# SynthAIr/T-VQ-VAE-TrajGen

Hardware: AMD Instinct MI355X
Metric: stage1+stage2 train steps/sec on synthetic (B,C,T) trajectories, 1/2/4/8 GPU (higher is better)
Workload: dtype fp32; 1 GPU; stage1 VQ-VAE + stage2 MaskGIT joint train step, per-GPU batch (B=256,C=6,T=256), K=512, configs/config.yaml architecture; global_batch=256, seq_len=256, parallelism=dp1, launch=hipgraph

## Files before the change

t-vq-vae-trajgen_amd/csrc/tvq_conv_wgrad.hip:

```cpp
#include "tvq_conv_core.h"
#include "tvq_conv_internal.h"
#include "tvq_gemm.h"
#include "tvq_reduce.h"

#include <algorithm>
#include <vector>

namespace tvq {

template <int KH, int KW, int SW, bool REPL, int TN, int TK, int WN, int WK>
__global__ __launch_bounds__(256) void conv_wgrad_kernel(const float* __restrict__ G,
                                                        const float* __restrict__ in,
                                                        float* __restrict__ slab, ConvGeom g,
                                                        int pos_per_split, int kcols) {
  constexpr int BK = 16;
  constexpr int KK = KH * KW;
  constexpr int FN = TN / WN / 16;
  constexpr int FK = TK / WK / 16;
  constexpr int SA = ((TN + 31) / 32) * 32 + 16;
  constexpr int SB = ((TK + 31) / 32) * 32 + 16;
  constexpr int A_PER = TN * BK / 256;
  constexpr int B_PER = TK * BK / 256;
  static_assert(A_PER >= 1 && B_PER >= 1, "tile too small");
  __shared__ float As[BK * SA];
  __shared__ float Bs[BK * SB];

  const int tid = threadIdx.x, lane = tid & 63, wid = tid >> 6;
  const int wn = wid % WN, wk = wid / WN;
  const int n0 = blockIdx.y * TN;
  const int kp0 = blockIdx.x * TK;
  const int p_begin = blockIdx.z * pos_per_split;
  const int p_end = min(g.Mpos, p_begin + pos_per_split);

  const int kk_t = tid % BK;
  const int a_nbase = tid / BK;
  const int b_kbase = tid / BK;
  int bc_off[B_PER], bkh[B_PER], bkw[B_PER];
  unsigned bmask = 0u, bones = 0u;
#pragma unroll
  for (int j = 0; j < B_PER; ++j) {
    const int kp = kp0 + b_kbase + j * 16;
    const int c = kp / KK, r = kp - c * KK;
    bkh[j] = r / KW - g.oph;
    bkw[j] = r - (r / KW) * KW - g.opw;
    bc_off[j] = (kp < g.Kred) ? c * g.Hin * g.Win : 0;
    if (kp < g.Kred) bmask |= 1u << j;
    if (kp == g.Kred && kp < kcols) bones |= 1u << j;
  }

  float ra[A_PER], rb[B_PER];
  auto load_tile = [&](int p0) {
    const int p = p0 + kk_t;
    const bool pv = p < p_end;
    int b = 0, h = 0, w = 0;
    if (pv) {
      const uint32_t bh = fdiv((uint32_t)p, g.fd_wo);
      w = p - (int)bh * g.Wo;
      b = (int)fdiv((uint32_t)p, g.fd_hwo);
      h = (int)bh - b * g.Hout;
    }
    const float* gb = G + (((int64_t)b * g.N) * g.Hout + h) * g.Wo + w;
#pragma unroll
    for (int j = 0; j < A_PER; ++j) {
      const int n = n0 + a_nbase + j * 16;
      ra[j] = (pv && n < g.N) ? gb[(int64_t)n * g.Hout * g.Wo] : 0.f;
    }
    const float* inb = in + (int64_t)b * g.C * g.Hin * g.Win;
#pragma unroll
    for (int j = 0; j < B_PER; ++j) {
      float v = (pv && (bones >> j & 1u)) ? 1.0f : 0.f;
      if (pv && (bmask >> j & 1u)) {
        int hi = h + bkh[j], wi = w * SW + bkw[j];
        bool ok = true;
        if (REPL) {
          hi = hi < 0 ? 0 : (hi >= g.Hin ? g.Hin - 1 : hi);
          wi = wi < 0 ? 0 : (wi >= g.Win ? g.Win - 1 : wi);
        } else {
          ok = hi >= 0 && hi < g.Hin && wi >= 0 && wi < g.Win;
        }
        if (ok) v = inb[bc_off[j] + (int64_t)hi * g.Win + wi];
      }
      rb[j] = v;
    }
  };
  auto store_tile = [&]() {
#pragma unroll
    for (int j = 0; j < A_PER; ++j) As[kk_t * SA + ((a_nbase + j * 16) ^ (kk_t & 14))] = ra[j];
#pragma unroll
    for (int j = 0; j < B_PER; ++j) Bs[kk_t * SB + ((b_kbase + j * 16) ^ (kk_t & 14))] = rb[j];
  };

  floatx4 acc[FN][FK];
#pragma unroll
  for (int i = 0; i < FN; ++i)
#pragma unroll
    for (int j = 0; j < FK; ++j) acc[i][j] = floatx4{0.f, 0.f, 0.f, 0.f};
  const int r16 = lane & 15, g4 = lane >> 4;
  if (p_begin < p_end) {
    load_tile(p_begin);
    for (int p0 = p_begin; p0 < p_end; p0 += BK) {
      __syncthreads();
      store_tile();
      __syncthreads();
      if (p0 + BK < p_end) load_tile(p0 + BK);
#pragma unroll
      for (int kk = 0; kk < BK; kk += 4) {
        float af[FN], bf[FK];
        const int swz = r16 ^ ((kk & 12) | (g4 & 2));
#pragma unroll
        for (int i = 0; i < FN; ++i) af[i] = As[(kk + g4) * SA + (wn * FN + i) * 16 + swz];
#pragma unroll
        for (int j = 0; j < FK; ++j) bf[j] = Bs[(kk + g4) * SB + (wk * FK + j) * 16 + swz];
#pragma unroll
        for (int i = 0; i < FN; ++i)
#pragma unroll
          for (int j = 0; j < FK; ++j) acc[i][j] = mfma16x16x4(af[i], bf[j], acc[i][j]);
      }
    }
  }
  float* sl = slab + (int64_t)blockIdx.z * g.N * kcols;
#pragma unroll
  for (int i = 0; i < FN; ++i)
#pragma unroll
    for (int j = 0; j < FK; ++j)
#pragma unroll
      for (int r = 0; r < 4; ++r) {
        const int n = n0 + (wn * FN + i) * 16 + 4 * g4 + r;
        const int kp = kp0 + (wk * FK + j) * 16 + r16;
        if (n < g.N && kp < kcols) sl[(int64_t)n * kcols + kp] = acc[i][j][r];
      }
}
__device__ __forceinline__ void chan_sum_final_one(const float* part, int chunks, int c,
                                                   float* out, int accumulate) {
  float s = 0.f;
  for (int i = 0; i < chunks; ++i) s += ld_wt(part + (int64_t)c * chunks + i);
  out[c] = accumulate ? out[c] + s : s;
}
__global__ __launch_bounds__(256) void chan_sum_partial_kernel(const float* __restrict__ x, int B,
                                                               int C, int HW, int ipc, int chunks,
                                                               int vec, float* __restrict__ part,
                                                               int* __restrict__ cnt,
                                                               float* __restrict__ out,
                                                               int accumulate) {
  __shared__ float red[4];
  const int c = blockIdx.x, ch = blockIdx.y;
  const int b0 = ch * ipc, b1 = min(B, b0 + ipc);
  float s = 0.f;
  if (vec) {
    const int hw4 = HW >> 2, n4 = (b1 - b0) * hw4;
    for (int i0 = threadIdx.x; i0 < n4; i0 += 256 * 4) {
      floatx4 v[4];
#pragma unroll
      for (int u = 0; u < 4; ++u) {
        const int i = i0 + u * 256;
        const int bb = b0 + (i < n4 ? i : 0) / hw4, q = (i < n4 ? i : 0) % hw4;
        v[u] = *reinterpret_cast<const floatx4*>(x + ((int64_t)bb * C + c) * HW + 4 * q);
      }
#pragma unroll
      for (int u = 0; u < 4; ++u)
        if (i0 + u * 256 < n4) s += (v[u][0] + v[u][1]) + (v[u][2] + v[u][3]);
    }
  } else {
    const int n = (b1 - b0) * HW;
    for (int i = threadIdx.x; i < n; i += 256) {
      const int bb = b0 + i / HW, p = i % HW;
      s += x[((int64_t)bb * C + c) * HW + p];
    }
  }
  s = block_sum(s, red);
  if (threadIdx.x == 0) st_wt(part + (int64_t)c * chunks + ch, s);
  if (cnt && last_block(cnt + c, chunks) && threadIdx.x < 64) {
    float t = threadIdx.x < chunks ? ld_wt(part + (int64_t)c * chunks + threadIdx.x) : 0.f;
    t = wave_sum(t);
    if (threadIdx.x == 0) out[c] = accumulate ? out[c] + t : t;
  }
}
__global__ void chan_sum_final_kernel(const float* __restrict__ part, int C, int chunks,
                                      float* __restrict__ out, int accumulate) {
  const int c = blockIdx.x * blockDim.x + threadIdx.x;
  if (c >= C) return;
  chan_sum_final_one(part, chunks, c, out, accumulate);
}

struct WHaloGeom {
  Div16 dv_hw, dv_wp, dv_gst;
  int B, C, Hin, Win, N, Hout, Wo;
  int oh, ow, HP, WP, PS;
  int P, GST, CB;
  int Kred, kcols;
  int ips;
};

template <int KH, int KW, int SW, bool REPL, int FN>
__global__ __launch_bounds__(256) void conv_wgrad_halo_kernel(const float* __restrict__ G,
                                                             const float* __restrict__ in,
                                                             float* __restrict__ slab,
                                                             WHaloGeom g) {
  constexpr int KK = KH * KW;
  constexpr int NB = FN * 16;
  extern __shared__ float smem[];
  float* Gs = smem;
  float* Hs = smem + NB * g.GST;
  const int tid = threadIdx.x, lane = tid & 63, wid = tid >> 6;
  const int s = blockIdx.x;
  const int n0 = blockIdx.y * NB;
  const int c0 = blockIdx.z * g.CB;
  const int cbn = min(g.CB, g.C - c0);
  const bool last_cb = c0 + g.CB >= g.C;
  const int kb = cbn * KK + ((last_cb && g.kcols > g.Kred) ? 1 : 0);
  const int KT = (kb + 15) / 16;
  const int j = lane & 15, kq = lane >> 4;

  for (int idx = tid; idx < g.PS; idx += 256) Hs[g.CB * g.PS + idx] = 1.0f;
  int koff[4];
#pragma unroll
  for (int t = 0; t < 4; ++t) {
    const int kl = (wid + 4 * t) * 16 + j;
    const int c = kl / KK, tap = kl - c * KK;
    koff[t] = kl < cbn * KK ? c * g.PS + (tap / KW) * g.WP + (tap % KW) : g.CB * g.PS;
  }
  const int ktw = wid < KT ? (KT - wid + 3) / 4 : 0;

  floatx4 acc[FN][4];
#pragma unroll
  for (int i = 0; i < FN; ++i)
#pragma unroll
    for (int t = 0; t < 4; ++t) acc[i][t] = floatx4{0.f, 0.f, 0.f, 0.f};

  const int b_begin = s * g.ips, b_end = min(g.B, b_begin + g.ips);
  for (int b = b_begin; b < b_end; ++b) {
    __syncthreads();
    const float* gb = G + ((int64_t)b * g.N + n0) * g.P;
    const int gtot = NB * g.GST;
    for (int base = tid; base < gtot; base += 256 * HALO_U) {
      float v[HALO_U];
#pragma unroll
      for (int u = 0; u < HALO_U; ++u) {
        const int idx = base + u * 256;
        const int nn = div16(idx, g.dv_gst), m = idx - nn * g.GST;
        v[u] = (idx < gtot && m < g.P && n0 + nn < g.N) ? gb[(int64_t)nn * g.P + m] : 0.f;
      }
#pragma unroll
      for (int u = 0; u < HALO_U; ++u)
        if (base + u * 256 < gtot) Gs[base + u * 256] = v[u];
    }
    halo_fill<GATHER_F, KH, KW, SW, REPL>(Hs, in + ((int64_t)b * g.C + c0) * g.Hin * g.Win, cbn,
                                          cbn, g.Hin, g.Win, g.HP, g.WP, g.PS, g.oh, g.ow,
                                          g.dv_hw, g.dv_wp, tid);
    __syncthreads();
    int h0 = 0, w0 = 0;
    for (int m0 = 0; m0 < g.P; m0 += 4) {
      const int base = h0 * g.WP + (w0 + kq) * SW;
      float af[FN];
#pragma unroll
      for (int i = 0; i < FN; ++i) af[i] = Gs[(i * 16 + j) * g.GST + m0 + kq];
#pragma unroll
      for (int t = 0; t < 4; ++t) {
        if (t < ktw) {
          const float bf = Hs[base + koff[t]];
#pragma unroll
          for (int i = 0; i < FN; ++i) acc[i][t] = mfma16x16x4(af[i], bf, acc[i][t]);
        }
      }
      w0 += 4;
      if (w0 == g.Wo) { w0 = 0; ++h0; }
    }
  }
  float* out = slab + (int64_t)s * g.N * g.kcols;
#pragma unroll
  for (int t = 0; t < 4; ++t) {
    if (t >= ktw) continue;
    const int kl = (wid + 4 * t) * 16 + j;
    int kg;
    if (kl < cbn * KK) kg = c0 * KK + kl;
    else if (kl == cbn * KK && kb > cbn * KK) kg = g.Kred;
    else continue;
#pragma unroll
    for (int i = 0; i < FN; ++i)
#pragma unroll
      for (int r = 0; r < 4; ++r) {
        const int n = n0 + i * 16 + kq * 4 + r;
        if (n < g.N) out[(int64_t)n * g.kcols + kg] = acc[i][t][r];
      }
  }
}

#ifndef TVQ_W8_IMG
#define TVQ_W8_IMG 16
#endif
constexpr int W8_IMG = TVQ_W8_IMG;
constexpr int W8_STG = 4;

struct W8Probs {
  const float* G[4];
  const float* X[4];
  float* slab[4];
};

template <int W, int CB>
__global__ __launch_bounds__(256) void conv_wgrad_w8_kernel(W8Probs pr, int B, int C, int N,
                                                           int kcols, int PS) {
  constexpr int P = 3 * W, WP = W + 2;
  constexpr int GST = P + 4;
  constexpr int KB = CB * 9 + 1, KT = (KB + 15) / 16;
  constexpr int TW = KT * 16;
  extern __shared__ float smem[];
  constexpr int STG = W8_STG, NSTG = W8_IMG / STG;
  static_assert(STG == 4 && W8_IMG % STG == 0, "one image per wave and stage");
  const int hs_img = (CB + 1) * PS;
  const int gbuf = STG * 32 * GST, hbuf = STG * hs_img;
  float* Gs = smem;
  float* Hs = smem + 2 * gbuf;
  const int tid = threadIdx.x, lane = tid & 63, wid = tid >> 6;
  const int j = lane & 15, kq = lane >> 4;
  const int nty = (N + 31) / 32, pb = (int)blockIdx.y / nty;
  const float* __restrict__ G = pr.G[pb];
  const float* __restrict__ X = pr.X[pb];
  float* __restrict__ slab = pr.slab[pb];
  const int s = blockIdx.x, n0 = ((int)blockIdx.y - pb * nty) * 32, c0 = blockIdx.z * CB;
  const bool bias = c0 + CB >= C && kcols > C * 9;
  const int b0 = s * W8_IMG;
  const int ni = min(W8_IMG, B - b0);
  constexpr int GQ = P / 4, GN = STG * 32 * GQ, GU = (GN + 255) / 256;
  constexpr int XQ = W / 4, XN = STG * CB * 3 * XQ, XU = (XN + 255) / 256;
  float4 gv[GU], xv[XU];
  auto load = [&](int sg) {
#pragma unroll
    for (int u = 0; u < GU; ++u) {
      const int e = tid + u * 256;
      const int ii = e / (32 * GQ), r = (e / GQ) % 32, q = e % GQ, im = sg * STG + ii;
      gv[u] = make_float4(0.f, 0.f, 0.f, 0.f);
      if (e < GN && im < ni && n0 + r < N)
        gv[u] = *reinterpret_cast<const float4*>(G + ((int64_t)(b0 + im) * N + n0 + r) * P + 4 * q);
    }
#pragma unroll
    for (int u = 0; u < XU; ++u) {
      const int e = tid + u * 256;
      const int ii = e / (CB * 3 * XQ), c = (e / (3 * XQ)) % CB, hq = e % (3 * XQ), im = sg * STG + ii;
      xv[u] = make_float4(0.f, 0.f, 0.f, 0.f);
      if (e < XN && im < ni && c0 + c < C)
        xv[u] = *reinterpret_cast<const float4*>(X + ((int64_t)(b0 + im) * C + c0 + c) * P + 4 * hq);
    }
  };
  auto store = [&](int buf) {
#pragma unroll
    for (int u = 0; u < GU; ++u) {
      const int e = tid + u * 256;
      if (e < GN) {
        const int ii = e / (32 * GQ), r = (e / GQ) % 32, q = e % GQ;
        *reinterpret_cast<float4*>(Gs + buf * gbuf + (ii * 32 + r) * GST + 4 * q) = gv[u];
      }
    }
#pragma unroll
    for (int u = 0; u < XU; ++u) {
      const int e = tid + u * 256;
      if (e < XN) {
        const int ii = e / (CB * 3 * XQ), c = (e / (3 * XQ)) % CB, hq = e % (3 * XQ);
        const int h = hq / XQ, q = hq % XQ;
        float* d = Hs + buf * hbuf + ii * hs_img + c * PS + (h + 1) * WP + 1 + 4 * q;
        d[0] = xv[u].x; d[1] = xv[u].y; d[2] = xv[u].z; d[3] = xv[u].w;
      }
    }
  };
  load(0);
  for (int e = tid; e < 2 * hbuf; e += 256) Hs[e] = (e % hs_img) >= CB * PS ? 1.f : 0.f;
  __syncthreads();
  store(0);
  __syncthreads();
  int koff[KT];
#pragma unroll
  for (int t = 0; t < KT; ++t) {
    const int kl = t * 16 + j, c = kl / 9, tap = kl - 9 * c;
    koff[t] = kl < CB * 9 ? c * PS + (tap / 3) * WP + (tap % 3) : CB * PS;
  }
  floatx4 acc[2][KT];
#pragma unroll
  for (int i = 0; i < 2; ++i)
#pragma unroll
    for (int t = 0; t < KT; ++t) acc[i][t] = floatx4{0.f, 0.f, 0.f, 0.f};
  for (int sg = 0; sg < NSTG; ++sg) {
    const int cur = sg & 1;
    if (sg + 1 < NSTG) load(sg + 1);
    if (sg * STG + wid < ni) {
      const float* gb = Gs + cur * gbuf + wid * 32 * GST + j * GST + kq;
      const float* hb = Hs + cur * hbuf + wid * hs_img + kq;
#pragma unroll
      for (int m0 = 0; m0 < P; m0 += 4) {
        const int base = (m0 / W) * WP + (m0 % W);
        const float a0 = gb[m0], a1 = gb[16 * GST + m0];
#pragma unroll
        for (int t = 0; t < KT; ++t) {
          const float bv = hb[base + koff[t]];
          acc[0][t] = mfma16x16x4(a0, bv, acc[0][t]);
          acc[1][t] = mfma16x16x4(a1, bv, acc[1][t]);
        }
      }
    }
    if (sg + 1 < NSTG) store(cur ^ 1);
    __syncthreads();
  }
  float* red = smem;
#pragma unroll
  for (int i = 0; i < 2; ++i)
#pragma unroll
    for (int t = 0; t < KT; ++t)
#pragma unroll
      for (int r = 0; r < 4; ++r) red[(wid * 32 + i * 16 + 4 * kq + r) * TW + t * 16 + j] = acc[i][t][r];
  __syncthreads();
  const int kb = CB * 9 + (bias ? 1 : 0);
  float* out = slab + (int64_t)s * N * kcols;
  for (int e = tid; e < 32 * kb; e += 256) {
    const int row = e / kb, col = e - row * kb;
    const int n = n0 + row;
    if (n >= N) continue;
    const float v = ((red[row * TW + col] + red[(32 + row) * TW + col]) +
                     red[(64 + row) * TW + col]) + red[(96 + row) * TW + col];
    const int kg = col < CB * 9 ? c0 * 9 + col : C * 9;
    out[(int64_t)n * kcols + kg] = v;
  }
}

template <int W, int CB>
static size_t w8_lds(int PS) {
  constexpr int P = 3 * W, GST = P + 4;
  const size_t a = (size_t)2 * W8_STG * 32 * GST + (size_t)2 * W8_STG * (CB + 1) * PS;
  const size_t red = (size_t)4 * 32 * (((CB * 9 + 1 + 15) / 16) * 16);
  return 4 * (a > red ? a : red);
}

static bool w8_fits(int64_t B, int64_t C, int64_t H, int64_t Wi, int64_t N, int64_t Wo, int64_t KH,
                    int64_t KW, int64_t SW, int64_t replicate) {
  return KH == 3 && KW == 3 && SW == 1 && !replicate && H == 3 && Wi == Wo &&
         Wi == 8 && N % 32 == 0 && C % 8 == 0 && B % W8_IMG == 0;
}
static int64_t w8_ws(int64_t B, int64_t N, int64_t C) {
  const int64_t S = B / W8_IMG, kc = C * 9 + 1;
  return S * N * kc + reduce_rows_scratch(S, N * kc);
}

constexpr int WT_T = 512, WT_AP = 128 + 4;
template <int KH, int KW>
struct WtCfg {
  static constexpr int KK = KH * KW, NCH = 128 / KK + 2;
  static constexpr int XROW = 34, XCH = KH * XROW;
  static constexpr int AS = 32 * WT_AP, XS = NCH * XCH;
  static constexpr int XPER = (XS + WT_T - 1) / WT_T;
  static_assert(XPER <= 32, "staging mask");
};

struct WtGeom {
  int B, C, N, H, W, Kred, kcols;
  int segs;
  int spr;
  int ntiles;
};

__device__ __forceinline__ int wt_crow(int r, int h) { return (r & 3) + 8 * (r >> 2) + 4 * h; }

template <int KH, int KW>
struct WtRegs {
  float4 ga[2];
  float xv[WtCfg<KH, KW>::XPER];
  uint32_t ok;
};

template <int KH, int KW>
__global__ __launch_bounds__(WT_T) void conv_wgrad_t32_kernel(const float* __restrict__ G,
                                                             const float* __restrict__ X,
                                                             float* __restrict__ slab, WtGeom g,
                                                             int ktiles) {
  using R = WtCfg<KH, KW>;
  using Regs = WtRegs<KH, KW>;
  constexpr int PH = KH / 2, PW = (KW - 1) / 2;
  __shared__ float As[2][R::AS];
  __shared__ float Xs[2][R::XS];
  const int tid = threadIdx.x, lane = tid & 63;
  const int wid = __builtin_amdgcn_readfirstlane(tid >> 6);
  const int wn = wid & 3, wk = wid >> 2;
  int z, tile;
  xcd_tile((int)blockIdx.x, ktiles * g.ntiles, &z, &tile);
  const int nst = g.B * g.H * g.segs;
  const int s_begin = z * g.spr, s_end = min(nst, s_begin + g.spr);
  if (s_begin >= nst) return;
  const int k0 = (tile % ktiles) * 128, n0 = (tile / ktiles) * 128;
  const int c_lo = k0 / R::KK;
  int boff[2];
#pragma unroll
  for (int j = 0; j < 2; ++j) {
    int kp = k0 + wk * 64 + j * 32 + (lane & 31);
    kp = kp < g.Kred ? kp : g.Kred - 1;
    const int c = kp / R::KK, t = kp - c * R::KK, kh = t / KW, kw = t - kh * KW;
    boff[j] = (c - c_lo) * R::XCH + kh * R::XROW + kw;
  }
  auto load = [&](Regs& q, int s) {
    if (s >= s_end) return;
    const int row = s / g.segs, w0 = (s - row * g.segs) * 32;
    const int b = row / g.H, h = row - b * g.H;
#pragma unroll
    for (int j = 0; j < 2; ++j) {
      const int e = tid + j * WT_T, n = e >> 3, p4 = (e & 7) * 4;
      const int nn = n0 + n < g.N ? n0 + n : g.N - 1;
      q.ga[j] = *(const float4*)(G + ((int64_t)(b * g.N + nn) * g.H + h) * g.W + w0 + p4);
    }
    q.ok = 0u;
#pragma unroll
    for (int u = 0; u < R::XPER; ++u) {
      const int e = tid + u * WT_T;
      const int c = e / R::XCH, r = e - c * R::XCH, kh = r / R::XROW, jj = r - kh * R::XROW;
      const int cc = c_lo + c, hi = h + kh - PH, wi = w0 - PW + jj;
      const bool ok = e < R::XS && cc < g.C && hi >= 0 && hi < g.H && wi >= 0 && wi < g.W;
      q.xv[u] = X[ok ? ((int64_t)(b * g.C + cc) * g.H + hi) * g.W + wi : 0];
      q.ok |= (ok ? 1u : 0u) << u;
    }
  };
  auto store = [&](const Regs& q, int buf) {
#pragma unroll
    for (int j = 0; j < 2; ++j) {
      const int e = tid + j * WT_T, n = e >> 3, p4 = (e & 7) * 4;
      float* d = As[buf] + p4 * WT_AP + n;
      d[0] = q.ga[j].x;
      d[WT_AP] = q.ga[j].y;
      d[2 * WT_AP] = q.ga[j].z;
      d[3 * WT_AP] = q.ga[j].w;
    }
#pragma unroll
    for (int u = 0; u < R::XPER; ++u) {
      const int e = tid + u * WT_T;
      if (e < R::XS) Xs[buf][e] = (q.ok >> u & 1u) ? q.xv[u] : 0.f;
    }
  };
  floatx16 acc[2];
#pragma unroll
  for (int j = 0; j < 2; ++j)
#pragma unroll
    for (int r = 0; r < 16; ++r) acc[j][r] = 0.f;
  float bsum = 0.f;
  auto body = [&](int s, const Regs& next, Regs& free) {
    const int buf = (s - s_begin) & 1;
    load(free, s + 2);
    const float* as = As[buf] + wn * 32 + (lane & 31);
    const float* xs = Xs[buf];
#pragma unroll
    for (int st = 0; st < 16; ++st) {
      const int p = 2 * st + (lane >> 5);
      const float a = as[p * WT_AP];
#pragma unroll
      for (int j = 0; j < 2; ++j)
        acc[j] = __builtin_amdgcn_mfma_f32_32x32x2f32(a, xs[boff[j] + p], acc[j], 0, 0, 0);
    }
    if (k0 == 0 && tid < 128) {
#pragma unroll 8
      for (int p = 0; p < 32; ++p) bsum += As[buf][p * WT_AP + tid];
    }
    if (s + 1 < s_end) store(next, buf ^ 1);
    __syncthreads();
  };
  Regs r0, r1;
  load(r0, s_begin);
  load(r1, s_begin + 1);
  store(r0, 0);
  __syncthreads();
  for (int s = s_begin; s < s_end; s += 2) {
    body(s, r1, r0);
    if (s + 1 < s_end) body(s + 1, r0, r1);
  }
  float* sl = slab + (int64_t)z * g.N * g.kcols;
#pragma unroll
  for (int j = 0; j < 2; ++j) {
    const int kp = k0 + wk * 64 + j * 32 + (lane & 31);
    if (kp >= g.Kred) continue;
#pragma unroll
    for (int r = 0; r < 16; ++r) {
      const int n = n0 + wn * 32 + wt_crow(r, lane >> 5);
      if (n < g.N) sl[(int64_t)n * g.kcols + kp] = acc[j][r];
    }
  }
  if (k0 == 0 && tid < 128 && g.kcols > g.Kred && n0 + tid < g.N)
    sl[(int64_t)(n0 + tid) * g.kcols + g.Kred] = bsum;
}

static bool wt32_fits(int64_t B, int64_t C, int64_t H, int64_t Wi, int64_t N, int64_t Wo,
                      int64_t KH, int64_t KW, int64_t SW, int64_t replicate) {
  return SW == 1 && !replicate && KW == 3 && (KH == 1 || KH == 3) && Wi == Wo &&
         Wi % 32 == 0 && N >= 64 && C >= 64 && B * C * H * Wi < (1ll << 31) &&
         B * N * H * Wo < (1ll << 31);
}
static void wt32_plan(int64_t B, int64_t C, int64_t H, int64_t W, int64_t N, int64_t KK,
                      int* S, int* spr) {
  const int64_t kt = (C * KK + 127) / 128, nt = (N + 127) / 128;
  const int64_t nst = B * H * (W / 32);
  int64_t s = (512 + kt * nt - 1) / (kt * nt);
  if (s > 256) s = 256;
  if (s > nst) s = nst;
  if (s < 1) s = 1;
  const int64_t per = (nst + s - 1) / s;
  *spr = (int)per;
  *S = (int)((nst + per - 1) / per);
}
static int64_t wt32_ws(int64_t B, int64_t C, int64_t H, int64_t W, int64_t N, int64_t KK) {
  int S, spr;
  wt32_plan(B, C, H, W, N, KK, &S, &spr);
  const int64_t kc = C * KK + 1;
  return (int64_t)S * N * kc + reduce_rows_scratch(S, N * kc);
}

struct WHaloPlan {
  WHaloGeom g;
  int FN, S, nblk, cblk;
  size_t lds;
};

static int64_t whalo_slab_max() { return (int64_t)(8 << 20); }

static int whalo_splits(int64_t N, int64_t C, int KK, int64_t B, int nblk, int cblk) {
  const int64_t kc = C * KK + 1;
  int64_t S = 1024 / (nblk * cblk);
  const int64_t cap = whalo_slab_max() / (N * kc);
  if (S > cap) S = cap;
  if (S > B) S = B;
  if (S < 1) S = 1;
  const int64_t ips = (B + S - 1) / S;
  return (int)((B + ips - 1) / ips);
}

static void whalo_blocking(int64_t N, int64_t C, int KK, int* FN, int* CB) {
  *FN = N <= 16 ? 1 : (N <= 32 ? 2 : 4);
  int cb = 1;
  while (cb * 2 <= C && (cb * 2) * KK + 1 <= 256) cb *= 2;
  if (cb > C) cb = (int)C;
  *CB = cb;
}

static int whalo_plane_stride(int hw, int KK, int KW, int WP, int SW, int CB) {
  int best = hw + ((16 - hw % 32) + 32) % 32, best_cost = 1 << 30;
  const int ncols = CB * KK;
  for (int pad = 0; pad < 32; ++pad) {
    const int PS = hw + pad;
    int cost = 0;
    for (int t0 = 0; t0 < ncols; t0 += 16) {
      int hits[32][2];
      int cnt[32] = {0};
      for (int l = 0; l < 32; ++l) {
        const int j = l & 15, kq = l >> 4;
        const int kl = t0 + j;
        if (kl >= ncols) continue;
        const int c = kl / KK, tap = kl - c * KK;
        const int a = c * PS + (tap / KW) * WP + (tap % KW) + kq * SW;
        const int bank = ((a % 32) + 32) % 32;
        bool dup = false;
        for (int q = 0; q < cnt[bank] && q < 2; ++q) dup |= hits[bank][q] == a;
        if (dup) continue;
        if (cnt[bank] < 2) hits[bank][cnt[bank]] = a;
        ++cnt[bank];
      }
      int worst = 0;
      for (int b = 0; b < 32; ++b) worst = cnt[b] > worst ? cnt[b] : worst;
      cost += worst > 1 ? worst - 1 : 0;
    }
    if (cost < best_cost) {
      best_cost = cost;
      best = PS;
    }
  }
  return best;
}

static bool whalo_plan(int B, int C, int Hin, int Win, int N, int Hout, int Wo, int KH, int KW,
                       int SW, int oh, int ow, int kcols, WHaloPlan* pl) {
  if (Wo % 4 != 0) return false;
  if (Hout * Wo > 128 && C > 64) return false;
  if ((int64_t)C * N >= 128 * 128) return false;
  WHaloGeom g;
  g.B = B; g.C = C; g.Hin = Hin; g.Win = Win; g.N = N; g.Hout = Hout; g.Wo = Wo;
  g.oh = oh; g.ow = ow;
  g.HP = Hout + KH - 1;
  g.WP = (Wo - 1) * SW + KW;
  const int hw = g.HP * g.WP;
  g.P = Hout * Wo;
  g.GST = g.P + ((2 - g.P % 32) + 32) % 32;
  if (g.WP < 2 || g.P >= (1 << 16)) return false;
  g.dv_hw = make_div16(hw);
  g.dv_wp = make_div16(g.WP);
  g.dv_gst = make_div16(g.GST);
  const int KK = KH * KW;
  int FN, CB;
  whalo_blocking(N, C, KK, &FN, &CB);
  g.PS = whalo_plane_stride(hw, KK, KW, g.WP, SW, CB);
  g.CB = CB;
  g.Kred = C * KK;
  g.kcols = kcols;
  const size_t fl = (size_t)FN * 16 * g.GST + (size_t)(CB + 1) * g.PS;
  if (fl * 4 > (size_t)HALO_LDS_MAX) return false;
  pl->nblk = (N + FN * 16 - 1) / (FN * 16);
  pl->cblk = (C + CB - 1) / CB;
  pl->S = whalo_splits(N, C, KK, B, pl->nblk, pl->cblk);
  g.ips = (B + pl->S - 1) / pl->S;
  pl->g = g;
  pl->FN = FN;
  pl->lds = fl * 4;
  return true;
}

template <int KH, int KW, int SW, bool REPL>
static void launch_wgrad_halo(const float* G, const float* in, float* slab, const WHaloPlan& pl,
                              hipStream_t st) {
  const dim3 grid(pl.S, pl.nblk, pl.cblk);
#define W_(FN_)                                                                              \
  hipLaunchKernelGGL((conv_wgrad_halo_kernel<KH, KW, SW, REPL, FN_>), grid, dim3(256), pl.lds, \
                     st, G, in, slab, pl.g)
  if (pl.FN == 1) W_(1); else if (pl.FN == 2) W_(2); else W_(4);
#undef W_
}

template <int KH, int KW, int SW, bool REPL>
static void launch_wgrad(const float* G, const float* in, float* slab, int splits, int pps,
                         const ConvGeom& g, int kcols, hipStream_t st) {
  if (g.N <= 16) {
    dim3 grid((kcols + 63) / 64, (g.N + 15) / 16, splits);
    hipLaunchKernelGGL((conv_wgrad_kernel<KH, KW, SW, REPL, 16, 64, 1, 4>), grid, dim3(256), 0, st,
                       G, in, slab, g, pps, kcols);
  } else {
    dim3 grid((kcols + 63) / 64, (g.N + 63) / 64, splits);
    hipLaunchKernelGGL((conv_wgrad_kernel<KH, KW, SW, REPL, 64, 64, 2, 2>), grid, dim3(256), 0, st,
                       G, in, slab, g, pps, kcols);
  }
}

static int wgrad_splits(const ConvGeom& g, int tiles, int* pps) {
  int splits = (1024 + tiles - 1) / tiles;
  const int maxs = (g.Mpos + 511) / 512;
  if (splits > maxs) splits = maxs;
  if (splits < 1) splits = 1;
  if (splits > 256) splits = 256;
  int per = (g.Mpos + splits - 1) / splits;
  per = (per + 15) / 16 * 16;
  splits = (g.Mpos + per - 1) / per;
  *pps = per;
  return splits;
}

struct RdRec {
  RrJob job;
  hipStream_t st;
};
static std::vector<RdRec> g_rd;
static bool g_rd_on = false, g_rd_paused = false;

static bool rd_records(int64_t rows) {
  return g_rd_on && !g_rd_paused && rows <= RR_ONE_ROWS;
}

static void wgrad_finish(float* slab, int splits, int64_t N, int64_t kcols, float* dw,
                         float* db, int accumulate, hipStream_t st) {
  const int64_t L = kcols > 0 && db ? kcols : 0;
  if (rd_records(splits)) {
    g_rd.push_back({{slab, dw, db, splits, N * kcols, L, accumulate}, st});
    return;
  }
  reduce_rows(slab, splits, N * kcols, N * kcols, dw, db, L, accumulate,
              slab + (int64_t)splits * N * kcols, st);
}

void param_rows_finish(const float* in, int64_t P, int64_t N, float* out, int accumulate,
                       float* scratch, hipStream_t st) {
  if (rd_records(P)) {
    g_rd.push_back({{in, out, nullptr, P, N, 0, accumulate}, st});
    return;
  }
  reduce_rows(in, P, N, N, out, nullptr, 0, accumulate, scratch, st);
}

void conv_wgrad_finish(float* slab, int splits, int64_t N, int64_t kcols, float* dw, float* db,
                       int accumulate, hipStream_t st) {
  wgrad_finish(slab, splits, N, kcols, dw, db, accumulate, st);
}

template <int W>
static void w8_launch_w(const W8Probs& pr, dim3 grid, int B, int C, int N, int kcols, int PS,
                        hipStream_t st) {
  static bool attr = false;
  if (!attr) {
    (void)hipFuncSetAttribute(reinterpret_cast<const void*>(&conv_wgrad_w8_kernel<W, 8>),
                              hipFuncAttributeMaxDynamicSharedMemorySize, 128 * 1024);
    attr = true;
  }
  hipLaunchKernelGGL((conv_wgrad_w8_kernel<W, 8>), grid, dim3(256), (w8_lds<W, 8>(PS)), st, pr, B,
                     C, N, kcols, PS);
}

template <typename... A>
static void w8_launch(int W, int n, const float* const* x, const float* const* dy, float* const* ws,
                      float* const* dw, float* const* db, int64_t B, int64_t C, int64_t N,
                      int kcols, int accumulate, hipStream_t st, const char* note, A... note_args) {
  const int S = (int)(B / W8_IMG);
  const int PS = whalo_plane_stride(5 * (W + 2), 9, 3, W + 2, 1, 8);
  const dim3 grid((unsigned)S, (unsigned)(n * (N / 32)), (unsigned)(C / 8));
  W8Probs pr = {};
  for (int i = 0; i < n; ++i) {
    pr.G[i] = dy[i];
    pr.X[i] = x[i];
    pr.slab[i] = ws[i];
  }
  TVQ_PLAN(note, note_args...);
  if (W == 8) w8_launch_w<8>(pr, grid, (int)B, (int)C, (int)N, kcols, PS, st);
  else w8_launch_w<16>(pr, grid, (int)B, (int)C, (int)N, kcols, PS, st);
  for (int i = 0; i < n; ++i) wgrad_finish(ws[i], S, N, kcols, dw[i], db[i], accumulate, st);
}

int64_t conv_wgrad_w16_slab_floats(int64_t B, int64_t C, int64_t N) {
  return (B / W8_IMG) * N * (C * 9 + 1);
}
bool conv_wgrad_w16_fits(int64_t B, int64_t C, int64_t N) {
  return B % W8_IMG == 0 && C % 8 == 0 && N % 32 == 0 && B > 0;
}
void conv_wgrad_w16_multi(int n, const float* const* x, const float* const* dy, float* const* ws,
                          float* const* dw, float* const* db, int64_t B, int64_t C, int64_t N,
                          int accumulate, hipStream_t st) {
  w8_launch(16, n, x, dy, ws, dw, db, B, C, N, (int)(C * 9 + 1), accumulate, st,
            "conv_wgrad_w16 n=%d S=%d", n, (int)(B / W8_IMG));
}
bool conv_wgrad_w8_fits(int64_t B, int64_t C, int64_t N) {
  return w8_fits(B, C, 3, 8, N, 8, 3, 3, 1, 0);
}
void conv_wgrad_w8_multi(int n, const float* const* x, const float* const* dy, float* const* ws,
                         float* const* dw, float* const* db, int64_t B, int64_t C, int64_t N,
                         int accumulate, hipStream_t st) {
  w8_launch(8, n, x, dy, ws, dw, db, B, C, N, (int)(C * 9 + 1), accumulate, st,
            "conv_wgrad_w8 n=%d S=%d", n, (int)(B / W8_IMG));
}
bool conv_wgrad_w8_pair(const float* x0, const float* dy0, float* ws0, float* dw0, float* db0,
                        const float* x1, const float* dy1, float* ws1, float* dw1, float* db1,
                        int64_t B, int64_t C, int64_t N, int accumulate, hipStream_t st) {
  if (!w8_fits(B, C, 3, 8, N, 8, 3, 3, 1, 0)) return false;
  const float* const x[2] = {x0, x1};
  const float* const dy[2] = {dy0, dy1};
  float* const ws[2] = {ws0, ws1};
  float* const dw[2] = {dw0, dw1};
  float* const db[2] = {db0, db1};
  w8_launch(8, 2, x, dy, ws, dw, db, B, C, N, (int)(C * 9 + 1), accumulate, st,
            "conv_wgrad_w8 pair S=%d", (int)(B / W8_IMG));
  return true;
}

static int64_t wgrad_ws(int64_t N, int64_t Kred, int64_t Mpos, int* splits_out, int* pps_out) {
  ConvGeom g;
  g.Mpos = (int)Mpos;
  const int64_t kc = Kred + 1;
  const int tiles = (int)(((kc + 63) / 64) * ((N + (N <= 16 ? 15 : 63)) / (N <= 16 ? 16 : 64)));
  int pps;
  const int splits = wgrad_splits(g, tiles, &pps);
  if (splits_out) *splits_out = splits;
  if (pps_out) *pps_out = pps;
  return (int64_t)splits * N * kc + reduce_rows_scratch(splits, N * kc);
}

static int64_t whalo_ws(int64_t N, int64_t C, int64_t KH, int64_t KW, int64_t B) {
  int FN, CB;
  const int KK = (int)(KH * KW);
  whalo_blocking(N, C, KK, &FN, &CB);
  const int nblk = (int)((N + FN * 16 - 1) / (FN * 16)), cblk = (int)((C + CB - 1) / CB);
  const int S = whalo_splits(N, C, KK, B, nblk, cblk);
  const int64_t kc = C * KK + 1;
  return (int64_t)S * N * kc + reduce_rows_scratch(S, N * kc);
}

int64_t conv_wgrad_ws(int64_t N, int64_t C, int64_t KH, int64_t KW, int64_t B, int64_t Hout,
                      int64_t Wo) {
  const int64_t a = wgrad_ws(N, C * KH * KW, B * Hout * Wo, nullptr, nullptr);
  const int64_t h = whalo_ws(N, C, KH, KW, B);
  const int64_t w = (KH == 3 && KW == 3 && B % W8_IMG == 0) ? w8_ws(B, N, C) : 0;
  const int64_t t = wt32_fits(B, C, Hout, Wo, N, Wo, KH, KW, 1, 0)
                        ? wt32_ws(B, C, Hout, Wo, N, KH * KW) : 0;
  const int64_t s2 = (KH == 3 && KW == 4 && C <= 16 && N <= 16) ? ws2_ws(B, C, Wo, N) : 0;
  return std::max(std::max(std::max(a, t), std::max(h, w)), s2);
}

}

using namespace tvq;

extern "C" int tvq_conv_wgrad_defer_begin(void) {
  TVQ_CHECK_ARG(!g_rd_on, "tvq_conv_wgrad_defer_begin: a scope is already open");
  g_rd.clear();
  g_rd_on = true;
  return TVQ_OK;
}

extern "C" int tvq_wgrad_defer_begin_stream(tvq_stream_t stream) {
  (void)stream;
  return tvq_conv_wgrad_defer_begin();
}

extern "C" int tvq_conv_wgrad_defer_pause(int64_t paused) {
  g_rd_paused = paused != 0;
  return TVQ_OK;
}

extern "C" int tvq_conv_wgrad_defer_flush(tvq_stream_t stream) {
  g_rd_on = false;
  g_rd_paused = false;
  (void)stream;
  std::vector<RrJob> jobs;
  while (!g_rd.empty()) {
    const hipStream_t st = g_rd.front().st;
    jobs.clear();
    std::vector<RdRec> rest;
    int64_t bytes = 0;
    for (const RdRec& r : g_rd) {
      if (r.st == st) {
        jobs.push_back(r.job);
        bytes += r.job.P * r.job.N * 4;
        TVQ_PLAN("wgrad_flush_job st=%p P=%lld N=%lld", (void*)st, (long long)r.job.P,
                 (long long)r.job.N);
      } else {
        rest.push_back(r);
      }
    }
    TVQ_PLAN("wgrad_flush st=%p jobs=%d MB=%.1f", (void*)st, (int)jobs.size(), bytes / 1e6);
    reduce_rows_batch(jobs.data(), (int)jobs.size(), st);
    g_rd.swap(rest);
  }
  return launch_status("tvq_conv_wgrad_defer_flush");
}

extern "C" int tvq_conv2d_wgrad(const float* x, int64_t B, int64_t Ci, int64_t H, int64_t Wi,
                                const float* dy, int64_t Co, int64_t Wo, int64_t KH, int64_t KW,
                                int64_t SW, int64_t replicate, float* dw, float* db,
                                int64_t accumulate, float* workspace, tvq_stream_t stream) {
  TVQ_CHECK_ARG(x && dy && dw && workspace, "tvq_conv2d_wgrad: bad arguments");
  const int kind = kind_of((int)KH, (int)KW, (int)SW);
  TVQ_CHECK_ARG(kind >= 0, "tvq_conv2d_wgrad: unsupported kernel");
  ConvGeom g = make_geom((int)B, (int)Ci, (int)H, (int)Wi, (int)Co, (int)H, (int)Wo, (int)KH,
                         (int)KW, PH_OF(KH), PW_OF(KW), Ci * KH * KW, KH * KW);
  const int kcols = g.Kred + (db ? 1 : 0);
  hipStream_t st = (hipStream_t)stream;
  if (ws2_fits(Ci, H, Co, KH, KW, SW)) {
    const int S = ws2_launch(dy, x, workspace, (int)B, (int)Ci, (int)Co, (int)Wi, (int)Wo, kcols,
                             replicate != 0, st);
    wgrad_finish(workspace, S, Co, kcols, dw, db, (int)accumulate, st);
    return launch_status("tvq_conv2d_wgrad(s2)");
  }
  if (wt32_fits(B, Ci, H, Wi, Co, Wo, KH, KW, SW, replicate)) {
    WtGeom t;
    t.B = (int)B; t.C = (int)Ci; t.N = (int)Co; t.H = (int)H; t.W = (int)Wi;
    t.Kred = g.Kred; t.kcols = kcols; t.segs = (int)(Wi / 32);
    int S;
    wt32_plan(B, Ci, H, Wi, Co, KH * KW, &S, &t.spr);
    const int kt = (g.Kred + 127) / 128;
    t.ntiles = (int)((Co + 127) / 128);
    const dim3 grid(xcd_grid(S, kt * t.ntiles));
    TVQ_PLAN("conv_wgrad_t32 S=%d", S);
    if (KH == 3)
      hipLaunchKernelGGL((conv_wgrad_t32_kernel<3, 3>), grid, dim3(WT_T), 0, st, dy, x, workspace, t,
                         kt);
    else
      hipLaunchKernelGGL((conv_wgrad_t32_kernel<1, 3>), grid, dim3(WT_T), 0, st, dy, x, workspace, t,
                         kt);
    wgrad_finish(workspace, S, Co, kcols, dw, db, (int)accumulate, st);
    return launch_status("tvq_conv2d_wgrad(t32)");
  }
  if (w8_fits(B, Ci, H, Wi, Co, Wo, KH, KW, SW, replicate)) {
    w8_launch(8, 1, &x, &dy, &workspace, &dw, &db, B, Ci, Co, kcols, (int)accumulate, st,
              "conv_wgrad_w8 S=%d", (int)(B / W8_IMG));
    return launch_status("tvq_conv2d_wgrad(w8)");
  }
  WHaloPlan pl;
  if ((conv_config().halo & 2) && whalo_plan((int)B, (int)Ci, (int)H, (int)Wi, (int)Co, (int)H,
                                             (int)Wo, (int)KH, (int)KW, (int)SW, PH_OF(KH),
                                             PW_OF(KW), kcols, &pl)) {
    TVQ_PLAN("conv_wgrad_halo S=%d", pl.S);
#define M_(a, b_, c, d) launch_wgrad_halo<a, b_, c, d>(dy, x, workspace, pl, st);
    TVQ_DISPATCH_KIND(kind, replicate, M_)
#undef M_
    wgrad_finish(workspace, pl.S, Co, kcols, dw, db, (int)accumulate, st);
    return launch_status("tvq_conv2d_wgrad(halo)");
  }
  int splits, pps;
  wgrad_ws(Co, g.Kred, g.Mpos, &splits, &pps);
  TVQ_PLAN("conv_wgrad split=%d", splits);
#define M_(a, b_, c, d) launch_wgrad<a, b_, c, d>(dy, x, workspace, splits, pps, g, kcols, st);
  TVQ_DISPATCH_KIND(kind, replicate, M_)
#undef M_
  wgrad_finish(workspace, splits, Co, kcols, dw, db, (int)accumulate, st);
  return launch_status("tvq_conv2d_wgrad");
}

extern "C" int tvq_convT2d_wgrad(const float* x, int64_t B, int64_t Ci, int64_t H, int64_t Wi,
                                 const float* dy, int64_t Co, int64_t Wo, int64_t KH, int64_t KW,
                                 int64_t SW, float* dw, int64_t accumulate, float* workspace,
                                 tvq_stream_t stream) {
  TVQ_CHECK_ARG(x && dy && dw && workspace, "tvq_convT2d_wgrad: bad arguments");
  const int kind = kind_of((int)KH, (int)KW, (int)SW);
  TVQ_CHECK_ARG(kind >= 0, "tvq_convT2d_wgrad: unsupported kernel");
  ConvGeom g = make_geom((int)B, (int)Co, (int)H, (int)Wo, (int)Ci, (int)H, (int)Wi, (int)KH,
                         (int)KW, PH_OF(KH), PW_OF(KW), Co * KH * KW, KH * KW);
  hipStream_t st = (hipStream_t)stream;
  if (ws2_fits(Co, H, Ci, KH, KW, SW)) {
    const int S = ws2_launch(x, dy, workspace, (int)B, (int)Co, (int)Ci, (int)Wo, (int)Wi, g.Kred,
                             false, st);
    wgrad_finish(workspace, S, Ci, g.Kred, dw, nullptr, (int)accumulate, st);
    return launch_status("tvq_convT2d_wgrad(s2)");
  }
  WHaloPlan pl;
  if ((conv_config().halo & 2) && whalo_plan((int)B, (int)Co, (int)H, (int)Wo, (int)Ci, (int)H, (int)Wi,
                                      (int)KH, (int)KW, (int)SW, PH_OF(KH), PW_OF(KW), g.Kred,
                                      &pl)) {
    TVQ_PLAN("conv_wgrad_halo S=%d", pl.S);
#define M_(a, b_, c, d) launch_wgrad_halo<a, b_, c, false>(x, dy, workspace, pl, st);
    TVQ_DISPATCH_KIND(kind, 0, M_)
#undef M_
    wgrad_finish(workspace, pl.S, Ci, g.Kred, dw, nullptr, (int)accumulate, st);
    return launch_status("tvq_convT2d_wgrad(halo)");
  }
  int splits, pps;
  wgrad_ws(Ci, g.Kred, g.Mpos, &splits, &pps);
  TVQ_PLAN("conv_wgrad split=%d", splits);
#define M_(a, b_, c, d) launch_wgrad<a, b_, c, false>(x, dy, workspace, splits, pps, g, g.Kred, st);
  TVQ_DISPATCH_KIND(kind, 0, M_)
#undef M_
  wgrad_finish(workspace, splits, Ci, g.Kred, dw, nullptr, (int)accumulate, st);
  return launch_status("tvq_convT2d_wgrad");
}

extern "C" int64_t tvq_channel_sum_workspace(int64_t B, int64_t C, int64_t HW) {
  if (HW == 1) {
    const int64_t r = reduce_rows_scratch(B, C);
    return r > 0 ? r : 1;
  }
  int64_t chunks = (B * HW + 8191) / 8192;
  if (chunks > 64) chunks = 64;
  if (chunks < 1) chunks = 1;
  return C * chunks;
}

extern "C" int tvq_channel_sum(const float* x, int64_t B, int64_t C, int64_t HW, float* out,
                               int64_t accumulate, float* workspace, tvq_stream_t stream) {
  TVQ_CHECK_ARG(x && out && workspace && B > 0 && C > 0 && HW > 0, "tvq_channel_sum: bad args");
  if (HW == 1) {
    reduce_rows(x, B, C, C, out, nullptr, 0, (int)accumulate, workspace, (hipStream_t)stream);
    return launch_status("tvq_channel_sum");
  }
  const int64_t chunks = tvq_channel_sum_workspace(B, C, HW) / C;
  hipStream_t st = (hipStream_t)stream;
  int* cnt = counters(C, FIN_REDUCE);
  const int64_t ipc = (B + chunks - 1) / chunks;
  const int64_t nch = (B + ipc - 1) / ipc;
  TVQ_CHECK_ARG(ipc * HW < (1ll << 31), "tvq_channel_sum: bad geometry");
  const int vec = (HW & 3) == 0 && ((uintptr_t)x & 15) == 0;
  hipLaunchKernelGGL(chan_sum_partial_kernel, dim3((int)C, (int)nch), dim3(256), 0, st, x,
                     (int)B, (int)C, (int)HW, (int)ipc, (int)nch, vec, workspace, cnt, out,
                     (int)accumulate);
  if (!cnt)
    hipLaunchKernelGGL(chan_sum_final_kernel, dim3((int)((C + 127) / 128)), dim3(128), 0, st,
                       workspace, (int)C, (int)nch, out, (int)accumulate);
  return launch_status("tvq_channel_sum");
}
```

Before: 254.7 steps/s.

## Generalize W8 wgrad kernel to strided 3x4, 1x1 and replicate-padded convs

Templates the per-image LDS-staged MFMA weight-gradient kernel over kernel shape, stride and replicate padding. It adds a w8g path for 3x4 stride-2 convs (W=8/16), 1x1 convs with 64-channel blocks, and the transposed-conv wgrad, ahead of the halo and generic split-GEMM paths. The aim is to cut the cost of the generic wgrad for these small-H shapes. It adds more kernel instantiations and replicate halo filling in LDS stores, and relies on the plan picking correct geometry for each shape.

```diff
diff --git a/t-vq-vae-trajgen_amd/csrc/tvq_conv_wgrad.hip b/t-vq-vae-trajgen_amd/csrc/tvq_conv_wgrad.hip
--- a/t-vq-vae-trajgen_amd/csrc/tvq_conv_wgrad.hip
+++ b/t-vq-vae-trajgen_amd/csrc/tvq_conv_wgrad.hip
@@ -297,16 +297,28 @@
   float* slab[4];
 };
 
-template <int W, int CB>
-__global__ __launch_bounds__(256) void conv_wgrad_w8_kernel(W8Probs pr, int B, int C, int N,
-                                                           int kcols, int PS) {
-  constexpr int P = 3 * W, WP = W + 2;
-  constexpr int GST = P + 4;
-  constexpr int KB = CB * 9 + 1, KT = (KB + 15) / 16;
+template <int KH, int KW, int SW, int W>
+struct W8Geo {
+  static constexpr int KK = KH * KW, PH = KH / 2, PW = (KW - 1) / 2;
+  static constexpr int P = 3 * W;
+  static constexpr int WP = (W - 1) * SW + KW, WI = WP - 2 * PW, HP = 3 + KH - 1;
+  static constexpr int GST = P + 4;
+  static_assert(W % 4 == 0 && WI % 4 == 0, "4 positions of a step lie in one row; 16-B loads");
+};
+
+template <int KH, int KW, int SW, bool REPL, int W, int CB>
+__device__ __forceinline__ void w8_block(const W8Probs& pr, int B, int C, int N, int kcols,
+                                         int PS, const int img) {
+  using Q = W8Geo<KH, KW, SW, W>;
+  constexpr int KK = Q::KK, PH = Q::PH, PW = Q::PW, P = Q::P, WP = Q::WP, WI = Q::WI;
+  constexpr int GST = Q::GST;
+  constexpr int KB = CB * KK + 1, KT = (KB + 15) / 16;
   constexpr int TW = KT * 16;
+  static_assert(!REPL || (PH == 1 && PW == 1), "replicate: one halo cell on every side");
   extern __shared__ float smem[];
-  constexpr int STG = W8_STG, NSTG = W8_IMG / STG;
+  constexpr int STG = W8_STG;
   static_assert(STG == 4 && W8_IMG % STG == 0, "one image per wave and stage");
+  const int NSTG = img / STG;
   const int hs_img = (CB + 1) * PS;
   const int gbuf = STG * 32 * GST, hbuf = STG * hs_img;
   float* Gs = smem;
@@ -318,11 +330,11 @@
   const float* __restrict__ X = pr.X[pb];
   float* __restrict__ slab = pr.slab[pb];
   const int s = blockIdx.x, n0 = ((int)blockIdx.y - pb * nty) * 32, c0 = blockIdx.z * CB;
-  const bool bias = c0 + CB >= C && kcols > C * 9;
-  const int b0 = s * W8_IMG;
-  const int ni = min(W8_IMG, B - b0);
+  const bool bias = c0 + CB >= C && kcols > C * KK;
+  const int b0 = s * img;
+  const int ni = min(img, B - b0);
   constexpr int GQ = P / 4, GN = STG * 32 * GQ, GU = (GN + 255) / 256;
-  constexpr int XQ = W / 4, XN = STG * CB * 3 * XQ, XU = (XN + 255) / 256;
+  constexpr int XQ = WI / 4, XN = STG * CB * 3 * XQ, XU = (XN + 255) / 256;
   float4 gv[GU], xv[XU];
   auto load = [&](int sg) {
 #pragma unroll
@@ -339,7 +351,7 @@
       const int ii = e / (CB * 3 * XQ), c = (e / (3 * XQ)) % CB, hq = e % (3 * XQ), im = sg * STG + ii;
       xv[u] = make_float4(0.f, 0.f, 0.f, 0.f);
       if (e < XN && im < ni && c0 + c < C)
-        xv[u] = *reinterpret_cast<const float4*>(X + ((int64_t)(b0 + im) * C + c0 + c) * P + 4 * hq);
+        xv[u] = *reinterpret_cast<const float4*>(X + ((int64_t)(b0 + im) * C + c0 + c) * (3 * WI) + 4 * hq);
     }
   };
   auto store = [&](int buf) {
@@ -357,8 +369,22 @@
       if (e < XN) {
         const int ii = e / (CB * 3 * XQ), c = (e / (3 * XQ)) % CB, hq = e % (3 * XQ);
         const int h = hq / XQ, q = hq % XQ;
-        float* d = Hs + buf * hbuf + ii * hs_img + c * PS + (h + 1) * WP + 1 + 4 * q;
+        float* d = Hs + buf * hbuf + ii * hs_img + c * PS + (h + PH) * WP + PW + 4 * q;
         d[0] = xv[u].x; d[1] = xv[u].y; d[2] = xv[u].z; d[3] = xv[u].w;
+        if constexpr (REPL) {
+          const int dr = h == 0 ? -WP : (h == 2 ? WP : 0);
+          if (dr != 0) {
+            d[dr] = xv[u].x; d[dr + 1] = xv[u].y; d[dr + 2] = xv[u].z; d[dr + 3] = xv[u].w;
+          }
+          if (q == 0) {
+            d[-1] = xv[u].x;
+            if (dr != 0) d[dr - 1] = xv[u].x;
+          }
+          if (q == XQ - 1) {
+            d[4] = xv[u].w;
+            if (dr != 0) d[dr + 4] = xv[u].w;
+          }
+        }
       }
     }
   };
@@ -370,8 +396,8 @@
   int koff[KT];
 #pragma unroll
   for (int t = 0; t < KT; ++t) {
-    const int kl = t * 16 + j, c = kl / 9, tap = kl - 9 * c;
-    koff[t] = kl < CB * 9 ? c * PS + (tap / 3) * WP + (tap % 3) : CB * PS;
+    const int kl = t * 16 + j, c = kl / KK, tap = kl - KK * c;
+    koff[t] = kl < CB * KK ? c * PS + (tap / KW) * WP + (tap % KW) : CB * PS;
   }
   floatx4 acc[2][KT];
 #pragma unroll
@@ -383,10 +409,10 @@
     if (sg + 1 < NSTG) load(sg + 1);
     if (sg * STG + wid < ni) {
       const float* gb = Gs + cur * gbuf + wid * 32 * GST + j * GST + kq;
-      const float* hb = Hs + cur * hbuf + wid * hs_img + kq;
+      const float* hb = Hs + cur * hbuf + wid * hs_img + kq * SW;
 #pragma unroll
       for (int m0 = 0; m0 < P; m0 += 4) {
-        const int base = (m0 / W) * WP + (m0 % W);
+        const int base = (m0 / W) * WP + (m0 % W) * SW;
         const float a0 = gb[m0], a1 = gb[16 * GST + m0];
 #pragma unroll
         for (int t = 0; t < KT; ++t) {
@@ -407,7 +433,7 @@
 #pragma unroll
       for (int r = 0; r < 4; ++r) red[(wid * 32 + i * 16 + 4 * kq + r) * TW + t * 16 + j] = acc[i][t][r];
   __syncthreads();
-  const int kb = CB * 9 + (bias ? 1 : 0);
+  const int kb = CB * KK + (bias ? 1 : 0);
   float* out = slab + (int64_t)s * N * kcols;
   for (int e = tid; e < 32 * kb; e += 256) {
     const int row = e / kb, col = e - row * kb;
@@ -415,16 +441,28 @@
     if (n >= N) continue;
     const float v = ((red[row * TW + col] + red[(32 + row) * TW + col]) +
                      red[(64 + row) * TW + col]) + red[(96 + row) * TW + col];
-    const int kg = col < CB * 9 ? c0 * 9 + col : C * 9;
+    const int kg = col < CB * KK ? c0 * KK + col : C * KK;
     out[(int64_t)n * kcols + kg] = v;
   }
 }
 
 template <int W, int CB>
+__global__ __launch_bounds__(256) void conv_wgrad_w8_kernel(W8Probs pr, int B, int C, int N,
+                                                           int kcols, int PS) {
+  w8_block<3, 3, 1, false, W, CB>(pr, B, C, N, kcols, PS, W8_IMG);
+}
+
+template <int KH, int KW, int SW, bool REPL, int W, int CB>
+__global__ __launch_bounds__(256) void conv_wgrad_w8g_kernel(W8Probs pr, int B, int C, int N,
+                                                            int kcols, int PS, int img) {
+  w8_block<KH, KW, SW, REPL, W, CB>(pr, B, C, N, kcols, PS, img);
+}
+
+template <int KH, int KW, int SW, int W, int CB>
 static size_t w8_lds(int PS) {
-  constexpr int P = 3 * W, GST = P + 4;
-  const size_t a = (size_t)2 * W8_STG * 32 * GST + (size_t)2 * W8_STG * (CB + 1) * PS;
-  const size_t red = (size_t)4 * 32 * (((CB * 9 + 1 + 15) / 16) * 16);
+  using Q = W8Geo<KH, KW, SW, W>;
+  const size_t a = (size_t)2 * W8_STG * 32 * Q::GST + (size_t)2 * W8_STG * (CB + 1) * PS;
+  const size_t red = (size_t)4 * 32 * (((CB * Q::KK + 1 + 15) / 16) * 16);
   return 4 * (a > red ? a : red);
 }
 
@@ -775,6 +813,42 @@
   wgrad_finish(slab, splits, N, kcols, dw, db, accumulate, st);
 }
 
+constexpr int W8G_LDS_MAX = 128 * 1024;
+struct W8gPlan {
+  int img, S, PS;
+  size_t lds;
+};
+static int w8g_img(int64_t KH, int64_t KW, int64_t Wo) {
+  if (KH == 3 && KW == 4) return Wo == 8 ? 8 : (Wo == 16 ? 4 : 0);
+  if (KH == 1 && KW == 1) return Wo == 8 ? 4 : 0;
+  return 0;
+}
+static bool w8g_plan(int64_t B, int64_t C, int64_t H, int64_t Wi, int64_t N, int64_t Wo, int64_t KH,
+                     int64_t KW, int64_t SW, W8gPlan* pl) {
+  const int img = w8g_img(KH, KW, Wo);
+  if (!img || H != 3 || N % 32 != 0 || B <= 0 || B % img != 0) return false;
+  if (KH == 3) {
+    if (SW != 2 || Wi != 2 * Wo || C % 8 != 0) return false;
+    const int WP = (int)Wi + 2;
+    pl->PS = whalo_plane_stride(5 * WP, 12, 4, WP, 2, 8);
+    pl->lds = Wo == 8 ? w8_lds<3, 4, 2, 8, 8>(pl->PS) : w8_lds<3, 4, 2, 16, 8>(pl->PS);
+  } else {
+    if (SW != 1 || Wi != Wo || C % 64 != 0) return false;
+    pl->PS = whalo_plane_stride(3 * (int)Wi, 1, 1, (int)Wi, 1, 64);
+    pl->lds = w8_lds<1, 1, 1, 8, 64>(pl->PS);
+  }
+  pl->img = img;
+  pl->S = (int)(B / img);
+  return pl->lds <= (size_t)W8G_LDS_MAX;
+}
+static int64_t w8g_ws(int64_t N, int64_t C, int64_t KH, int64_t KW, int64_t B, int64_t Hout,
+                      int64_t Wo) {
+  const int img = w8g_img(KH, KW, Wo);
+  if (!img || Hout != 3 || B % img != 0) return 0;
+  const int64_t S = B / img, kc = C * KH * KW + 1;
+  return S * N * kc + reduce_rows_scratch(S, N * kc);
+}
+
 template <int W>
 static void w8_launch_w(const W8Probs& pr, dim3 grid, int B, int C, int N, int kcols, int PS,
                         hipStream_t st) {
@@ -784,8 +858,43 @@
                               hipFuncAttributeMaxDynamicSharedMemorySize, 128 * 1024);
     attr = true;
   }
-  hipLaunchKernelGGL((conv_wgrad_w8_kernel<W, 8>), grid, dim3(256), (w8_lds<W, 8>(PS)), st, pr, B,
-                     C, N, kcols, PS);
+  hipLaunchKernelGGL((conv_wgrad_w8_kernel<W, 8>), grid, dim3(256), (w8_lds<3, 3, 1, W, 8>(PS)),
+                     st, pr, B, C, N, kcols, PS);
+}
+
+template <int KH, int KW, int SW, bool REPL, int W, int CB>
+static void w8g_launch_k(const W8Probs& pr, const W8gPlan& pl, int B, int C, int N, int kcols,
+                         hipStream_t st) {
+  static bool attr = false;
+  if (!attr) {
+    (void)hipFuncSetAttribute(
+        reinterpret_cast<const void*>(&conv_wgrad_w8g_kernel<KH, KW, SW, REPL, W, CB>),
+        hipFuncAttributeMaxDynamicSharedMemorySize, W8G_LDS_MAX);
+    attr = true;
+  }
+  const dim3 grid((unsigned)pl.S, (unsigned)(N / 32), (unsigned)(C / CB));
+  hipLaunchKernelGGL((conv_wgrad_w8g_kernel<KH, KW, SW, REPL, W, CB>), grid, dim3(256), pl.lds, st,
+                     pr, B, C, N, kcols, pl.PS, pl.img);
+}
+
+static void w8g_launch(const W8gPlan& pl, const float* G, const float* in, float* ws, float* dw,
+                       float* db, int64_t B, int64_t C, int64_t N, int64_t Wo, int KH, int KW,
+                       int SW, bool repl, int kcols, int accumulate, hipStream_t st) {
+  W8Probs pr = {};
+  pr.G[0] = G;
+  pr.X[0] = in;
+  pr.slab[0] = ws;
+  TVQ_PLAN("conv_wgrad_w8 k%dx%d s%d repl=%d W=%d img=%d S=%d", KH, KW, SW, (int)repl, (int)Wo,
+           pl.img, pl.S);
+#define G_(KH_, KW_, SW_, R_, W_, CB_) \
+  w8g_launch_k<KH_, KW_, SW_, R_, W_, CB_>(pr, pl, (int)B, (int)C, (int)N, kcols, st)
+  if (KH == 1) G_(1, 1, 1, false, 8, 64);
+  else if (Wo == 8 && repl) G_(3, 4, 2, true, 8, 8);
+  else if (Wo == 8) G_(3, 4, 2, false, 8, 8);
+  else if (repl) G_(3, 4, 2, true, 16, 8);
+  else G_(3, 4, 2, false, 16, 8);
+#undef G_
+  wgrad_finish(ws, pl.S, N, kcols, dw, db, accumulate, st);
 }
 
 template <typename... A>
@@ -872,7 +981,8 @@
   const int64_t t = wt32_fits(B, C, Hout, Wo, N, Wo, KH, KW, 1, 0)
                         ? wt32_ws(B, C, Hout, Wo, N, KH * KW) : 0;
   const int64_t s2 = (KH == 3 && KW == 4 && C <= 16 && N <= 16) ? ws2_ws(B, C, Wo, N) : 0;
-  return std::max(std::max(std::max(a, t), std::max(h, w)), s2);
+  const int64_t wg = w8g_ws(N, C, KH, KW, B, Hout, Wo);
+  return std::max(std::max(std::max(a, t), std::max(h, w)), std::max(s2, wg));
 }
 
 }
@@ -964,6 +1074,12 @@
               "conv_wgrad_w8 S=%d", (int)(B / W8_IMG));
     return launch_status("tvq_conv2d_wgrad(w8)");
   }
+  W8gPlan gp;
+  if (w8g_plan(B, Ci, H, Wi, Co, Wo, KH, KW, SW, &gp)) {
+    w8g_launch(gp, dy, x, workspace, dw, db, B, Ci, Co, Wo, (int)KH, (int)KW, (int)SW,
+               replicate != 0, kcols, (int)accumulate, st);
+    return launch_status("tvq_conv2d_wgrad(w8g)");
+  }
   WHaloPlan pl;
   if ((conv_config().halo & 2) && whalo_plan((int)B, (int)Ci, (int)H, (int)Wi, (int)Co, (int)H,
                                              (int)Wo, (int)KH, (int)KW, (int)SW, PH_OF(KH),
@@ -1001,6 +1117,12 @@
     wgrad_finish(workspace, S, Ci, g.Kred, dw, nullptr, (int)accumulate, st);
     return launch_status("tvq_convT2d_wgrad(s2)");
   }
+  W8gPlan gp;
+  if (w8g_plan(B, Co, H, Wo, Ci, Wi, KH, KW, SW, &gp)) {
+    w8g_launch(gp, x, dy, workspace, dw, nullptr, B, Co, Ci, Wi, (int)KH, (int)KW, (int)SW, false,
+               g.Kred, (int)accumulate, st);
+    return launch_status("tvq_convT2d_wgrad(w8g)");
+  }
   WHaloPlan pl;
   if ((conv_config().halo & 2) && whalo_plan((int)B, (int)Co, (int)H, (int)Wo, (int)Ci, (int)H, (int)Wi,
                                       (int)KH, (int)KW, (int)SW, PH_OF(KH), PW_OF(KW), g.Kred,
```

New measurement: 255.9 steps/s, median of 6. No clear change (+0.5%).
